# GlassyWing/yolo_deepsort

Measured on AMD Instinct MI355X. Metric: end-to-end frames/sec (detect+ReID+assoc), 608x608, higher is better.
Workload: dtype f16x3

## Files before the change

### include/ydsort.h

```cpp
#ifndef YDSORT_H
#define YDSORT_H

#include <stddef.h>
#include <stdint.h>

#ifdef __cplusplus
extern "C" {
#endif

typedef struct yds_net yds_net;
typedef struct yds_reid yds_reid;
typedef struct yds_trk yds_trk;
typedef struct yds_pipe yds_pipe;
typedef struct yds_zones yds_zones;
typedef struct yds_act yds_act;
typedef struct yds_ident yds_ident;
typedef struct yds_comm yds_comm;

int yds_init(int device_id);
int yds_current_device(void);
int yds_device_pci_bus_id(char *buf, int len);
const char *yds_last_error(void);
int yds_device_count(void);
const char *yds_build_info(void);
// ... 119 lines not shown
yds_pipe *yds_pipeline_create_multi(yds_net *, yds_reid *, yds_trk *const *trks, int n_streams, float conf_thres, float nms_thres,
                                    const int32_t *class_mask, int n_mask);
int yds_pipeline_step_multi(yds_pipe *, const uint8_t *frames_dev, const uint8_t *next_frames_dev, int h, int w, int n_frames,
                            const int32_t *stream_of_frame, int32_t *out6_host, int cap, int32_t *counts_host);
int yds_pipeline_step_multi_host(yds_pipe *, const uint8_t *frames_host, const uint8_t *next_frames_host, int h, int w, int n_frames,
                                 const int32_t *stream_of_frame, int32_t *out6_host, int cap, int32_t *counts_host);
int yds_pipeline_step_multi_mixed(yds_pipe *, const uint8_t *frames_dev, const uint8_t *next_frames_dev, const uint64_t *frame_off,
                                  const int32_t *frame_hw , size_t frames_bytes, int n_frames,
                                  const int32_t *stream_of_frame, int32_t *out6_host, int cap, int32_t *counts_host);
int yds_pipeline_step_multi_mixed_host(yds_pipe *, const uint8_t *frames_host, const uint8_t *next_frames_host, const uint64_t *frame_off,
                                       const int32_t *frame_hw , size_t frames_bytes, int n_frames,
                                       const int32_t *stream_of_frame, int32_t *out6_host, int cap, int32_t *counts_host);
int yds_pipeline_prefetch_host(yds_pipe *, const uint8_t *frames_host, int h, int w, int batch);
int yds_pipeline_set_schedule(yds_pipe *, int min_crops);
int yds_pipeline_set_frame_order(yds_pipe *, int bgr);
int yds_pipeline_set_windows(yds_pipe *, int win_w, int win_h, double overlap);
int yds_pipeline_set_stream_windows(yds_pipe *, int stream, int win_w, int win_h, double overlap);
int yds_pipeline_last_schedule(yds_pipe *);
int yds_pipeline_schedule_trial(yds_pipe *, int uploaded, int *decided, double *serialized_s, double *two_stream_s);
int yds_pipeline_stage_us(yds_pipe *, float *us5);
int yds_overlay_tracks(const uint8_t *frames_dev, const int32_t *src_slot_host, int n_out, int h, int w, const int32_t *boxes_host,
                       const int32_t *box_ptr_host, const uint8_t *text_host, int n_text, const int32_t *fps_host,
                       const uint8_t *font_host, int n_glyphs, int thickness, int scale, uint8_t *out_dev, uint8_t *out_host);
int yds_swap_rb(uint8_t *frames_dev, size_t pixels);
int yds_overlay_tracks_bgr(uint8_t *frames_bgr_dev, int n_src, const int32_t *src_slot_host, int n_out, int h, int w, const int32_t *boxes_host,
                           const int32_t *box_ptr_host, const uint8_t *text_host, int n_text, const int32_t *fps_host,
                           const uint8_t *font_host, int n_glyphs, int thickness, int scale, uint8_t *out_host);
int yds_conv_timing(yds_net *, int mode, double *total_us, int64_t *launches, double *flops);
int yds_conv_timing_ex(yds_net *, int mode, double *total_us, int64_t *launches, double *flops, double *bytes, double *attainable_us);
int yds_conv_num_variants(void);
// ... 102 lines not shown
```

### yolo_deepsort_amd/_lib.py

```python

from __future__ import annotations

import ctypes as C
import os

import numpy as np

HERE = os.path.dirname(os.path.abspath(__file__))
_TAG = os.environ.get("YDS_BUILD_TAG", "")
LIB_PATH = os.path.join(HERE, "libydsort" + ("_" + _TAG if _TAG else "") + ".so")


class YdsError(RuntimeError):
    pass


_P = C.c_void_p
_I = C.c_int
_F = C.c_float
_SZ = C.c_size_t
_I64 = C.c_int64

SIGNATURES = {
    "yds_init": (_I, [_I]),
# ... 99 lines not shown
    "yds_pipeline_step_host": (_I, [_P, _P, _P, _I, _I, _I, _P, _I, _P]),
    "yds_pipeline_create_multi": (_P, [_P, _P, _P, _I, _F, _F, _P, _I]),
    "yds_pipeline_step_multi": (_I, [_P, _P, _P, _I, _I, _I, _P, _P, _I, _P]),
    "yds_pipeline_step_multi_host": (_I, [_P, _P, _P, _I, _I, _I, _P, _P, _I, _P]),
    "yds_pipeline_prefetch_host": (_I, [_P, _P, _I, _I, _I]),
    "yds_pipeline_set_next_injection": (_I, [_P, _I]),
    "yds_pipeline_stage_us": (_I, [_P, _P]),
    "yds_pipeline_set_schedule": (_I, [_P, _I]),
    "yds_pipeline_last_schedule": (_I, [_P]),
    "yds_pipeline_schedule_trial": (_I, [_P, _I, _P, _P, _P]),
    "yds_conv_timing": (_I, [_P, _I, _P, _P, _P]),
    "yds_overlay_tracks": (_I, [_P, _P, _I, _I, _I, _P, _P, _P, _I, _P, _P, _I, _I, _I, _P, _P]),
    "yds_swap_rb": (_I, [_P, _SZ]),
    "yds_overlay_tracks_bgr": (_I, [_P, _I, _P, _I, _I, _I, _P, _P, _P, _I, _P, _P, _I, _I, _I, _P]),
    "yds_pipeline_set_frame_order": (_I, [_P, _I]),
    "yds_pipeline_set_windows": (_I, [_P, _I, _I, C.c_double]),
    "yds_darknet_forward_u8_mixed_dev": (_I, [_P, _P, _P, _P, _SZ, _I]),
    "yds_reid_preprocess_mixed": (_I, [_P, _P, _P, _P, _I, _SZ, _P, _P, _I, _P]),
    "yds_reid_embed_mixed": (_I, [_P, _P, _P, _P, _I, _SZ, _P, _P, _I, _I, _P]),
    "yds_reid_front_fused": (_I, [_P]),
    "yds_reid_front_grid_crops": (_I, []),
    "yds_pipeline_step_multi_mixed": (_I, [_P, _P, _P, _P, _P, _SZ, _I, _P, _P, _I, _P]),
    "yds_pipeline_step_multi_mixed_host": (_I, [_P, _P, _P, _P, _P, _SZ, _I, _P, _P, _I, _P]),
    "yds_nms_ragged_pred": (_I, [_P, _SZ, _I, _I, _P, _P, _P, _P, _F, _F, _P, _I, _P]),
    "yds_pipeline_set_stream_windows": (_I, [_P, _I, _I, _I, C.c_double]),
    "yds_pipeline_slot_pred": (_I, [_P, _P, _SZ, _P]),
    "yds_gallery_search": (_I, [_P, _I, _P, _I, _I, _I, _F, _I, _P, _P, _P, _P]),
    "yds_gallery_search_dense": (_I, [_P, _I, _P, _I, _I, _P, _P, _P, _P, _I, _P]),
    "yds_gallery_link": (_I, [_P, _I, _I, _I, _I, _I, _F, _I, _P, _P, _P, _P]),
    "yds_tracker_get_gallery": (_I, [_P, _I, _P, _I, _P]),
# ... 193 lines not shown
```

### yolo_deepsort_amd/csrc/common.h

```cpp
#pragma once
#include <hip/hip_runtime.h>
#include <stdint.h>
#include <stdio.h>
#include <string>
#include <vector>
#include <stdexcept>

#include "slot_plan.h"

namespace yds {

void set_error(const std::string &msg);
struct Error : std::runtime_error {
    explicit Error(const std::string &m) : std::runtime_error(m) {}
};
[[noreturn]] void fail(const char *fmt, ...);
int bound_device();
void bind_thread();
hipStream_t make_stream(bool latency_role);

#define YDS_HIP(expr)                                                                          \
    do {                                                                                       \
        hipError_t _e = (expr);                                                                \
        if (_e != hipSuccess)                                                                  \
// ... 84 lines not shown
const char *conv_variant_name(int v);
double conv_flops(const ConvArgs &a);
double conv_bytes_io(const View &v);
double conv_bytes(const ConvArgs &a);

void launch_maxpool(const View &x, const View &y, int k, int stride, int pad, bool zero_pad_br, hipStream_t s);
void launch_upsample(const View &x, const View &y, int stride, hipStream_t s);
void launch_copy(const View &x, const View &y, hipStream_t s);
void launch_add(const View &a, const View &b, const View &y, hipStream_t s);
void launch_nchw_to_nhwc(const float *src_nchw, const View &y, int c_src, hipStream_t s);
void launch_nhwc_to_nchw(const View &x, float *dst_nchw, hipStream_t s);
void nhwc_to_host(const View &x, float *dst_nchw_host, hipStream_t s);
void launch_pack_h16(const float *src_f32, const View &y, hipStream_t s);
void launch_yolo_decode(const View &head, float *out, int total_boxes, int box_off, int num_classes,
                        const float *anchors_wh , int A, int img_h, int img_w, hipStream_t s);
void launch_inject(const View &head, int image, const float *rows_dev, int n, int head_index, int num_classes,
                   float logit, hipStream_t s);
void launch_inject_batch(const View &head, int batch, const float *table_dev, const int *offsets_dev, int max_rows, int head_index,
                         int num_classes, float logit, hipStream_t s);
void launch_resize_u8(const uint8_t *frames, int n, int h, int w, const View &y, hipStream_t s, bool bgr = false);
std::vector<FrameGeom> checked_layout(const uint64_t *frame_off, const int32_t *frame_hw, int n, size_t frames_bytes);
void launch_slot_resize(const uint8_t *frames, const SlotRec *slots, int n, const View &y, hipStream_t s, bool bgr);
void launch_slot_boxes(const float *pred, int n_boxes, int attrs, const SlotRec *slots, int n, float *dst, hipStream_t s);
struct ReidFront {
    const uint8_t *frames = nullptr;
    const FrameGeom *geom = nullptr;
    const int *boxes = nullptr;
    int h = 0, w = 0, bgr = 0;
};
void launch_crop_resize(const ReidFront &f, int D, const View &y, hipStream_t s);
// ... 7 lines not shown
```

### yolo_deepsort_amd/csrc/darknet.cpp

```cpp
#include "engine.h"
#include "h16.h"
#include "conv_common.h"

#include <math.h>
#include <stdlib.h>
#include <string.h>
#include <map>
#include <sstream>

namespace yds {

std::vector<CfgBlock> parse_cfg(const std::string &text) {
    std::vector<CfgBlock> blocks;
    std::istringstream in(text);
    std::string line;
    auto strip = [](std::string s) {
        size_t a = s.find_first_not_of(" \t\r\n"), b = s.find_last_not_of(" \t\r\n");
        return a == std::string::npos ? std::string() : s.substr(a, b - a + 1);
    };
    while (std::getline(in, line)) {
        if (line.empty() || line[0] == '#') continue;
        line = strip(line);
        if (line.empty()) fail("cfg: whitespace-only line (the reference parser rejects it too)");
        if (line[0] == '[') {
// ... 466 lines not shown
        l.tuned_batch = batch;
        l.tuned_math = mode;
    };
    for (const Step &st : plan(batch).steps) {
        if (st.kind > Step::CONV_BLOCK1) continue;
        if (st.kind == Step::CONV_STEM2 || st.kind == Step::CONV_BLOCK1) tune(st.layer - 1, false);
        tune(st.layer, st.kind == Step::CONV_MERGED);
    }
}

void Darknet::check_pass(int batch) const {
    if (batch < 1 || batch > batch_max) fail("forward: batch %d outside [1,%d]", batch, batch_max);
    if (math != conv_math()) fail("forward: this network was planned for conv math %d, current mode is %d (re-create it)", math, conv_math());
}

void Darknet::run_graph(int batch) {
    check_pass(batch);
    int lanes = getenv("YDS_DET_LANES") ? atoi(getenv("YDS_DET_LANES")) : 1;
    while (lanes > 1 && batch / lanes < 4) --lanes;
    if (lanes < 1) lanes = 1;
    if (lanes == 1) { run_lane(0, batch, stream); return; }
    while ((int)lane_streams.size() < lanes - 1) {
        hipStream_t st; hipEvent_t ev;
        YDS_HIP(hipStreamCreateWithFlags(&st, hipStreamNonBlocking));
        YDS_HIP(hipEventCreateWithFlags(&ev, hipEventDisableTiming));
        lane_streams.push_back(st); lane_done.push_back(ev);
    }
    if (!lane_fork) YDS_HIP(hipEventCreateWithFlags(&lane_fork, hipEventDisableTiming));
    const int per = (batch + lanes - 1) / lanes;
    YDS_HIP(hipEventRecord(lane_fork, stream));
    for (int k = 0; k < lanes; ++k) {
        const int first = k * per, cnt = std::min(per, batch - first);
        if (cnt <= 0) break;
        hipStream_t st = (k == 0 || time_convs) ? stream : lane_streams[k - 1];
        if (st != stream) YDS_HIP(hipStreamWaitEvent(st, lane_fork, 0));
        run_lane(first, cnt, st);
        if (st != stream) {
            YDS_HIP(hipEventRecord(lane_done[k - 1], st));
            YDS_HIP(hipStreamWaitEvent(stream, lane_done[k - 1], 0));
        }
    }
}

int Darknet::head_layers() const {
    double total = 0, acc = 0;
    for (int i = 0; i < (int)layers.size(); ++i)
        if (layers[i].type == L_CONV) total += conv_flops(conv_args(i, 1));
    for (int i = 0; i < (int)layers.size(); ++i) {
        if (layers[i].type != L_CONV) continue;
        acc += conv_flops(conv_args(i, 1));
        if (acc >= 0.06 * total) return i + 1;
    }
    return (int)layers.size();
}

bool Darknet::forward_resized_part(int batch, int part) {
    check_pass(batch);
    if (getenv("YDS_DET_LANES") && atoi(getenv("YDS_DET_LANES")) > 1) return false;
    const int cut = head_layers();
    if (part == 0) run_lane(0, batch, stream, 0, cut);
    else run_lane(0, batch, stream, cut, -1);
    return true;
}

void Darknet::enqueue_conv(const Step &st, int first, int batch, hipStream_t stream) {
    const int i = st.layer;
    const Layer &l = layers[i];
    if (!l.cw.loaded()) fail("forward: layer %d has no weights (call load_darknet_weights)", i);
    const ConvArgs a = conv_args(i, batch, first, st.kind == Step::CONV_MERGED);
    ConvTimeRec rec;
    if (time_convs) { rec.e0 = timing_event(); rec.e1 = timing_event(); YDS_HIP(hipEventRecord(rec.e0, stream)); }
    int variant;
    double extra_flops = 0, extra_bytes = 0;
    if (st.kind == Step::CONV_STEM2) {
        const ConvArgs a0 = conv_args(i - 1, batch, first);
        ConvKernelArgs k0 = make_conv_args(a0), k1 = make_conv_args(a);
// ... 13 lines not shown
        extra_bytes = conv_bytes(a2) - conv_bytes_io(a2.y) - conv_bytes_io(a.x) - (a.res.p ? conv_bytes_io(a.res) : 0.0);
    } else {
        variant = launch_conv(a, stream, l.variant);
    }
    if (time_convs) {
        YDS_HIP(hipEventRecord(rec.e1, stream));
        rec.variant = variant;
        rec.flops = conv_flops(a) + extra_flops;
        rec.bytes = conv_bytes(a) + extra_bytes;
        const double peak = conv_math() == MATH_F32 ? 157.3e12 : (a.terms == 1 ? 2500e12 : 2500e12 / 3);
        rec.attain_us = std::max(rec.flops / peak, rec.bytes / 6.29e12) * 1e6;
        conv_pending.push_back(rec);
    }
}

void Darknet::run_lane(int first, int batch, hipStream_t stream, int l0, int l1) {
    autotune(batch);
    if (l1 < 0) l1 = (int)layers.size();
    auto v = [&](int layer) { return view(layer, batch, first); };
    for (const Step &st : plan(batch).steps) {
        const int i = st.layer;
        if (i < l0) continue;
        if (i >= l1) break;
        const Layer &l = layers[i];
        switch (st.kind) {
        case Step::CONV: case Step::CONV_MERGED: case Step::CONV_STEM2: case Step::CONV_BLOCK1:
            enqueue_conv(st, first, batch, stream);
            break;
        case Step::MAXPOOL: launch_maxpool(v(st.src), v(i), st.ksize, st.stride, st.pad, st.zero_br, stream); break;
        case Step::UPSAMPLE: launch_upsample(v(l.src), v(i), l.stride, stream); break;
        case Step::COPY: {
// ... 1 lines not shown
            d.p += fmt_slots(d.fmt, st.arg);
            launch_copy(v(st.src), d, stream);
            break;
        }
        case Step::ADD: launch_add(v(l.refs[0]), v(l.refs[1]), v(i), stream); break;
        case Step::YOLO: {
            const View head = v(l.src);
            const int hidx = st.arg;
            if (inject_active && inject_set >= 0) {
                launch_inject_batch(head, batch, inject_table.p, inject_offsets_dev.p + (size_t)inject_set * batch_max + first, inject_max_rows, hidx,
                                    l.classes, inject_logit, stream);
            } else {
                for (int b = 0; b < batch && inject_active; ++b)
                    launch_inject(head, b, inject_rows[first + b].p, inject_n[first + b], hidx, l.classes, inject_logit, stream);
            }
            launch_yolo_decode(head, out.p + (size_t)first * total_boxes * attrs, total_boxes, l.box_off, l.classes, l.anchors.data(), (int)l.anchors.size() / 2, img_h, img_w, stream);
            break;
        }
        }
    }
}

void Darknet::forward_f32_host(const float *nchw, int batch, float *out_host) {
    size_t n = (size_t)batch * in_channels * img_h * img_w;
    YDS_HIP(hipMemcpyAsync(stage_f32.p, nchw, n * sizeof(float), hipMemcpyHostToDevice, stream));
    launch_nchw_to_nhwc(stage_f32.p, input_view(batch), in_channels, stream);
    run_graph(batch);
    if (out_host) YDS_HIP(hipMemcpyAsync(out_host, out.p, (size_t)batch * total_boxes * attrs * sizeof(float), hipMemcpyDeviceToHost, stream));
    YDS_HIP(hipStreamSynchronize(stream));
}

// ... 291 lines not shown
```

### yolo_deepsort_amd/csrc/engine.h

```cpp
#pragma once
#include "common.h"
#include "conv_weights.h"

#include <map>
#include <memory>
#include <string>
#include <utility>
#include <vector>

namespace yds {

struct CfgBlock {
    std::string type;
    std::map<std::string, std::string> kv;
};
std::vector<CfgBlock> parse_cfg(const std::string &text);

enum LayerType { L_CONV, L_MAXPOOL, L_UPSAMPLE, L_ROUTE, L_SHORTCUT, L_YOLO };

struct Layer {
    LayerType type = L_CONV;
    int c = 0, h = 0, w = 0;
    int root = -1, coff = 0;
    int src = -1;
// ... 26 lines not shown
    std::vector<Step> steps;
    std::vector<int> produced_by;
    int batch = -1, math = -1, epoch = -1;
};

struct Storage {
    DevBuf<float> buf;
    int ld = 0;
    int fmt = 0;
    int fmt_half = 0;
    bool owns = false;
    bool redirected = false;
    int into = -1, coff = 0;
};

class Darknet {
public:
    Darknet(const std::string &cfg_text, int img_h, int img_w, int batch_max);
    ~Darknet();
    void load_weights(const void *blob, size_t nbytes, int cutoff);
    void set_batch_max(int b);
    void forward_f32_host(const float *nchw, int batch, float *out_host);
    void forward_u8_host(const uint8_t *frames, int h, int w, int batch, float *out_host);
    void forward_u8_dev(const uint8_t *frames_dev, int h, int w, int batch);
    void forward_u8_frames_dev(const uint8_t *frames_dev, const std::vector<FrameGeom> &geom);
    void forward_resized(int batch) { run_graph(batch); }
    bool forward_resized_part(int batch, int part);
    int head_layers() const;
    void forward_tiles_host(const uint8_t *frame, int h, int w, const int *tiles_xyhw, int n_tiles);
    void forward_slots(const uint8_t *frames_dev, const SlotRec *slots, int n_slots, float *pred, bool bgr);
    void layer_output_host(int layer, int batch, float *nchw);
    void get_input_host(int batch, float *nchw);
    void set_injection(int image, const float *rows, int n, float logit);
    void load_injection_sets(const float *rows, const int *offsets, int n_sets, float logit);
    void select_injection_set(int set);
    void enable_conv_timing(bool on);
    void autotune(int batch);
    int64_t flops_per_image() const;
    View view(int layer, int batch, int first = 0) const;
    View input_view(int batch, int first = 0) const;
    ConvArgs conv_args(int layer, int batch, int first = 0, bool merged = false) const;

// ... 22 lines not shown
    int inject_max_rows = 0;
    int inject_set = -1;
    float inject_logit = 6.f;
    struct ConvTimeRec { hipEvent_t e0 = nullptr, e1 = nullptr; int variant = 0; double flops = 0, bytes = 0, attain_us = 0; };
    bool time_convs = false;
    std::vector<ConvTimeRec> conv_pending;
    std::vector<hipEvent_t> ev_pool;
    hipEvent_t timing_event();
    void resolve_conv_timing();
    double conv_us[kConvVariants] = {}, conv_flops_acc[kConvVariants] = {}, conv_bytes_acc[kConvVariants] = {}, conv_attain_us[kConvVariants] = {};
    int64_t conv_launches[kConvVariants] = {};

private:
    void allocate_buffers();
    void check_pass(int batch) const;
    void run_graph(int batch);
    void run_lane(int first, int batch, hipStream_t st, int l0 = 0, int l1 = -1);
    void enqueue_conv(const Step &st, int first, int batch, hipStream_t s);
    const LaunchPlan &plan(int batch);
    LaunchPlan plan_;
    int plan_epoch = 0;
    bool stem_fusable = false;
    int block1_at = -1;
    std::vector<hipStream_t> lane_streams;
    std::vector<hipEvent_t> lane_done;
    hipEvent_t lane_fork = nullptr;
};

struct NmsUniform { int32_t n_boxes, corner, merge; float sx, sy; };
class NmsWorkspace {
public:
    explicit NmsWorkspace(int max_candidates = 16384, int frames = 1);
    ~NmsWorkspace();
    NmsWorkspace(const NmsWorkspace &) = delete;
    void launch(const float *pred_dev, const NmsUniform &u, int n_frames, int attrs, float conf_thres, float iou_thres, int cap, hipStream_t s);
    void launch(const float *pred_dev, const NmsFrame *fr, int n_frames, int max_rows, size_t total_rows, int attrs, float conf_thres,
                float iou_thres, int cap, hipStream_t s);
    int collect(int frame, float *out6_host, int cap);
    void resize(int max_candidates, int n_frames);
    int needed(int n_frames) const;
    static constexpr int kMaxCandidates = 1 << 18;
    int run(const float *pred_dev, int n_boxes, int attrs, float conf_thres, float iou_thres, float sx, float sy,
            float *out6_host, int cap, hipStream_t s);
    int run_merge(const float *pred_dev, int n_boxes, int attrs, float conf_thres, float iou_thres, float *out6_host, int cap, hipStream_t s);
    int max_cand, frames;
    DevBuf<float> cand;
    DevBuf<float> sorted;
    DevBuf<int> counts;
    DevBuf<int> box_count;
    DevBuf<unsigned long long> mask;
    DevBuf<float> kept;
    int *h_counts = nullptr;
// ... 117 lines not shown
```

### yolo_deepsort_amd/csrc/layers.hip

```cpp
#include "common.h"

#include <algorithm>
#include "h16.h"
#include "resize_dev.h"

namespace yds {

static inline int grid_for(size_t work, int block = 256) {
    size_t g = (work + block - 1) / block;
    if (g > 8192) g = 8192;
    if (g < 1) g = 1;
    return (int)g;
}

__global__ void maxpool_kernel(const float *x, float *y, int N, int H, int W, int C, int ldx, int Ho, int Wo, int ldy,
                               int k, int stride, int pad, int zero_br, int fmt_in, int fmt_out) {
    fp16_saturate_on();
    const int C4 = C >> 2;
    const size_t total = (size_t)N * Ho * Wo * C4;
    for (size_t idx = blockIdx.x * (size_t)blockDim.x + threadIdx.x; idx < total; idx += (size_t)gridDim.x * blockDim.x) {
        int c4 = idx % C4;
        size_t pix = idx / C4;
        int ox = pix % Wo;
        size_t t = pix / Wo;
// ... 153 lines not shown
    if (y.c % 32 || y.ld % 32) fail("pack_h16: channels must be a multiple of 32");
    hipLaunchKernelGGL(pack_h16_kernel, dim3(grid_for(y.pixels() * (y.c / 4))), dim3(256), 0, s, src_f32, y.p, y.pixels(), y.c, y.ld);
    YDS_HIP(hipGetLastError());
}

void launch_nhwc_to_nchw(const View &x, float *dst_nchw, hipStream_t s) {
    hipLaunchKernelGGL(nhwc_to_nchw_kernel, dim3(grid_for(x.pixels() * x.c)), dim3(256), 0, s, x.p, dst_nchw, x.n, x.c, x.h, x.w, x.ld, x.fmt);
    YDS_HIP(hipGetLastError());
}

struct YoloParams {
    float aw[8], ah[8];
    float s0, s1;
};

__global__ void yolo_decode_kernel(const float *head, float *out, int N, int H, int W, int ld, int A, int attrs, int total_boxes,
                                   int box_off, YoloParams yp) {
    const int HW = H * W, n = blockIdx.y, per_cell = A * attrs;
    (void)N;
    const int lane = threadIdx.x & 63;
    const int wave0 = __builtin_amdgcn_readfirstlane((int)((blockIdx.x * blockDim.x + threadIdx.x) >> 6));
    const int nwaves = (int)((gridDim.x * blockDim.x) >> 6);
    for (int cell = wave0; cell < HW; cell += nwaves) {
        const int gy = cell / W, gx = cell - gy * W;
        const float *src = head + ((size_t)(n * H + gy) * W + gx) * ld;
        float *dst = out + ((size_t)n * total_boxes + box_off + cell) * attrs;
        for (int i = lane; i < per_cell; i += 64) {
            int a = 0;
#pragma unroll
            for (int k = 1; k < 8; ++k) a += (k < A && i >= k * attrs) ? 1 : 0;
            const int t = i - a * attrs;
            const float v = src[i];
            float r;
            if (t == 0) r = __fmul_rn(__fadd_rn(1.f / (1.f + expf(-v)), (float)gx), yp.s0);
            else if (t == 1) r = __fmul_rn(__fadd_rn(1.f / (1.f + expf(-v)), (float)gy), yp.s1);
            else if (t == 2) r = __fmul_rn(__fmul_rn(expf(v), yp.aw[a]), yp.s0);
            else if (t == 3) r = __fmul_rn(__fmul_rn(expf(v), yp.ah[a]), yp.s1);
            else r = 1.f / (1.f + expf(-v));
            dst[(size_t)a * HW * attrs + t] = r;
        }
    }
}

void launch_yolo_decode(const View &head, float *out, int total_boxes, int box_off, int num_classes, const float *anchors_wh,
                        int A, int img_h, int img_w, hipStream_t s) {
    if (A > 8) fail("yolo: at most 8 anchors per head");
    YoloParams yp;
    yp.s0 = (float)((double)img_h / head.h);
    yp.s1 = (float)((double)img_w / head.w);
    for (int a = 0; a < A; ++a) {
        yp.aw[a] = anchors_wh[2 * a] / yp.s0;
        yp.ah[a] = anchors_wh[2 * a + 1] / yp.s1;
    }
    int attrs = num_classes + 5;
    if (head.c != A * attrs) fail("yolo: head has %d channels, expected %d", head.c, A * attrs);
    const size_t per_img = (size_t)A * head.h * head.w * attrs;
    if (per_img >= (1ull << 31)) fail("yolo: head too large for 32-bit indexing");
    const unsigned cells = (unsigned)head.h * head.w;
    hipLaunchKernelGGL(yolo_decode_kernel, dim3(std::min((cells + 3) / 4, 2048u), head.n), dim3(256), 0, s, head.p, out, head.n, head.h, head.w,
                       head.ld, A, attrs, total_boxes, box_off, yp);
    YDS_HIP(hipGetLastError());
}

__global__ void inject_clear_kernel(float *head, int image, int H, int W, int ld, int A, int attrs, float logit) {
    int total = H * W * A;
    for (int idx = blockIdx.x * blockDim.x + threadIdx.x; idx < total; idx += gridDim.x * blockDim.x) {
        int a = idx % A, cell = idx / A;
        head[((size_t)image * H * W + cell) * ld + a * attrs + 4] = -logit;
    }
}
__device__ __forceinline__ bool inject_row_superseded(const float *rows, int r, int n) {
    const float *row = rows + (size_t)r * 9;
    for (int j = r + 1; j < n; ++j) {
        const float *o = rows + (size_t)j * 9;
        if (o[0] == row[0] && o[1] == row[1] && o[2] == row[2] && o[3] == row[3]) return true;
// ... 202 lines not shown
```

### yolo_deepsort_amd/csrc/nms.hip

```cpp
#include "engine.h"

#include <string.h>

#include <vector>

namespace yds {

constexpr int MAX_DET = 300;

__device__ __forceinline__ NmsFrame frame_at(const NmsUniform &u, int f) {
    return NmsFrame{(uint64_t)f * u.n_boxes, u.n_boxes, u.corner, u.merge, u.sx, u.sy, 0};
}
__device__ __forceinline__ NmsFrame frame_at(const NmsFrame *fr, int f) { return fr[f]; }

__device__ __forceinline__ void nms_count_body(const float *pred, int n_boxes, int attrs, float thr, int *box_count) {
    int i = blockIdx.x * blockDim.x + threadIdx.x;
    if (i >= n_boxes) return;
    const float *p = pred + (size_t)i * attrs;
    int cnt = 0;
    float obj = p[4];
    if (obj > thr) {
        for (int j = 5; j < attrs; ++j) cnt += __fmul_rn(p[j], obj) > thr;
    }
    box_count[i] = cnt;
// ... 244 lines not shown
    if (!frame_at(frames, blockIdx.x).merge) return;
    nms_merge_body(cand_all, sorted_all, counts_all, max_cand, iou_thres, kept_all);
}

__global__ __launch_bounds__(256) void nms_publish_kernel(const int *counts, const float *kept, int *h_counts, float *h_kept, int cap) {
    const int f = blockIdx.x;
    if (threadIdx.x < 4) h_counts[f * 4 + threadIdx.x] = counts[f * 4 + threadIdx.x];
    const int n = min(counts[f * 4 + 1], cap) * 6;
    const float *src = kept + (size_t)f * MAX_DET * 6;
    float *dst = h_kept + (size_t)f * MAX_DET * 6;
    for (int i = threadIdx.x; i < n; i += 256) dst[i] = src[i];
}

template <class Frames>
static void launch_stages(NmsWorkspace &w, const float *pred_dev, Frames frames, int n_frames, int max_rows, size_t total_rows, bool merge, int attrs,
                          float conf_thres, float iou_thres, int cap, hipStream_t s) {
    if (attrs < 6) fail("nms: predictions need at least one class");
    if (n_frames < 1 || max_rows < 1) fail("nms: %d frames of at most %d rows", n_frames, max_rows);
    if (n_frames > w.frames) w.resize(w.max_cand, n_frames);
    w.box_count.ensure(total_rows);
    const int nb = (max_rows + 255) / 256, max_cand = w.max_cand, words_ld = max_cand / 64;
    hipLaunchKernelGGL(nms_count_kernel<Frames>, dim3(nb, n_frames), dim3(256), 0, s, pred_dev, frames, attrs, conf_thres, w.box_count.p);
    hipLaunchKernelGGL(nms_scan_kernel<Frames>, dim3(1, n_frames), dim3(1024), 0, s, w.box_count.p, frames, w.counts.p);
    hipLaunchKernelGGL(nms_emit_kernel<Frames>, dim3(nb, n_frames), dim3(256), 0, s, pred_dev, frames, attrs, conf_thres, w.box_count.p, max_cand,
                       w.cand.p);
    hipLaunchKernelGGL(nms_rank_kernel, dim3(16, n_frames), dim3(256), 0, s, w.cand.p, w.counts.p, max_cand, w.sorted.p);
    hipLaunchKernelGGL(nms_mask_kernel, dim3(64, n_frames), dim3(256), 0, s, w.sorted.p, w.counts.p, max_cand, (double)iou_thres, w.mask.p, words_ld);
    hipLaunchKernelGGL(nms_sweep_kernel<Frames>, dim3(1, n_frames), dim3(256), words_ld * sizeof(unsigned long long), s, w.sorted.p, w.mask.p, words_ld,
                       w.counts.p, max_cand, frames, w.kept.p, cap);
    if (merge)
        hipLaunchKernelGGL(nms_merge_kernel<Frames>, dim3(n_frames), dim3(256), 0, s, w.cand.p, w.sorted.p, w.counts.p, max_cand, iou_thres, frames,
                           w.kept.p);
    hipLaunchKernelGGL(nms_publish_kernel, dim3(n_frames), dim3(256), 0, s, w.counts.p, w.kept.p, w.h_counts, w.h_kept, std::min(cap, (int)MAX_DET));
    YDS_HIP(hipGetLastError());
}

void NmsWorkspace::launch(const float *pred_dev, const NmsUniform &u, int n_frames, int attrs, float conf_thres, float iou_thres, int cap,
                          hipStream_t s) {
    launch_stages(*this, pred_dev, u, n_frames, u.n_boxes, (size_t)std::max(frames, n_frames) * u.n_boxes, u.merge != 0, attrs, conf_thres,
                  iou_thres, cap, s);
}

void NmsWorkspace::launch(const float *pred_dev, const NmsFrame *fr, int n_frames, int max_rows, size_t total_rows, int attrs, float conf_thres,
                          float iou_thres, int cap, hipStream_t s) {
    launch_stages(*this, pred_dev, fr, n_frames, max_rows, total_rows, true, attrs, conf_thres, iou_thres, cap, s);
}

template <class Launch> static void launch_grown(NmsWorkspace &w, int n_frames, hipStream_t s, Launch launch) {
    launch();
    YDS_HIP(hipStreamSynchronize(s));
    if (w.needed(n_frames) <= w.max_cand) return;
    w.resize(w.needed(n_frames), w.frames);
    launch();
    YDS_HIP(hipStreamSynchronize(s));
}

int NmsWorkspace::collect(int frame, float *out6_host, int cap) {
    const int *c = h_counts + frame * 4;
    if (c[0] > max_cand) fail("nms: %d candidates exceed the workspace capacity %d (caller must resize and relaunch)", c[0], max_cand);
    int n = c[1] < cap ? c[1] : cap;
// ... 113 lines not shown
```

### yolo_deepsort_amd/csrc/pipeline.cpp

```cpp
#include "engine.h"

#include <limits.h>
#include <stdlib.h>
#include <string.h>

#include <algorithm>
#include <chrono>
#include <utility>

namespace yds {

struct DetSlot {
    std::unique_ptr<NmsWorkspace> nms;
    hipEvent_t e0, e1, e2, e_nms;
    hipEvent_t e_r0, e_r1;
    bool reid_in_pass = false;
    DetSlot() { for (hipEvent_t *e : {&e0, &e1, &e2, &e_nms, &e_r0, &e_r1}) YDS_HIP(hipEventCreate(e)); }
    ~DetSlot() {
        for (hipEvent_t e : {e0, e1, e2, e_nms, e_r0, e_r1}) (void)hipEventDestroy(e);
        if (plan_tab) (void)hipHostFree(plan_tab);
    }
    void *plan_tab = nullptr;
    size_t plan_bytes = 0, plan_slots_n = 0;
    const SlotRec *plan_slots() const { return static_cast<const SlotRec *>(plan_tab); }
// ... 164 lines not shown
        p.split = false;
        if (!p.plan.empty()) s.write_plan(p.plan);
        if (p.plan.windowed) {
            YDS_HIP(hipEventRecord(s.e1, net->stream));
            return;
        }
        if (p.plan.direct()) launch_slot_resize(p.frames, s.plan_slots(), p.batch, net->input_view(p.batch), net->stream, frames_bgr);
        else launch_resize_u8(p.frames, p.batch, p.geo.h, p.geo.w, net->input_view(p.batch), net->stream, frames_bgr);
        YDS_HIP(hipEventRecord(s.e1, net->stream));
        stager.mark_read(p.frames, net->stream, FrameStager::DET);
        p.split = split && net->forward_resized_part(p.batch, 0);
    }
    void launch_detector_tail(Pass &p) {
        DetSlot &s = det[p.slot];
        const size_t per_slot = (size_t)net->total_boxes * net->attrs, n_slots = p.plan.slots.size();
        if (p.plan.windowed) {
            if (win_pred.n < n_slots * per_slot) {
                YDS_HIP(hipStreamSynchronize(net->stream));
                win_pred.alloc(n_slots * per_slot);
            }
            pred_rows = n_slots * net->total_boxes;
            net->forward_slots(p.frames, s.plan_slots(), (int)n_slots, win_pred.p, frames_bgr);
            stager.mark_read(p.frames, net->stream, FrameStager::DET);
        } else if (p.split) {
            (void)net->forward_resized_part(p.batch, 1);
        } else {
            net->forward_resized(p.batch);
        }
        YDS_HIP(hipEventRecord(s.e2, net->stream));
        if (p.plan.empty()) {
            const float sx = box_scale(p.geo.w, net->img_w), sy = box_scale(p.geo.h, net->img_h);
            s.nms->launch(net->out.p, NmsUniform{net->total_boxes, 0, 0, sx, sy}, p.batch, net->attrs, conf, nms_thres, 300, net->stream);
        } else {
            s.nms->launch(p.plan.windowed ? win_pred.p : net->out.p, s.plan_frames(), p.batch, p.plan.max_rows, n_slots * net->total_boxes,
                          net->attrs, conf, nms_thres, 300, net->stream);
        }
        YDS_HIP(hipEventRecord(s.e_nms, net->stream));
        p.done = Pass::WHOLE;
    }

    void set_windows(int ww, int wh, double overlap) {
        if (pending.frames || ahead.reid_in_flight) fail("pipeline: set_windows while a look-ahead pass is in flight (consume it with a step first)");
        if (ww > 0 && wh <= 0) fail("pipeline: window %d x %d", ww, wh);
        if (ww > 0 && !(overlap >= 0)) fail("pipeline: window overlap %g", overlap);
        if (ww > 0 && any_stream_windows()) fail("pipeline: set_windows while a stream holds a window setting of its own (set_stream_windows): one or the other");
        win_w = ww > 0 ? ww : 0; win_h = ww > 0 ? wh : 0; win_overlap = overlap;
    }
    bool any_stream_windows() const {
        for (const WindowSetting &sw : stream_win)
            if (sw.w > 0) return true;
        return false;
    }
    void set_stream_windows(int stream, int ww, int wh, double overlap) {
        if (!multi) fail("pipeline: created by yds_pipeline_create: it has no streams (window mode: yds_pipeline_set_windows)");
        if (stream < 0 || stream >= (int)trks.size()) fail("pipeline: stream %d outside [0,%zu)", stream, trks.size());
        if (ww > 0 && wh <= 0) fail("pipeline: window %d x %d", ww, wh);
        if (ww > 0 && !(overlap >= 0)) fail("pipeline: window overlap %g", overlap);
        if (pending.frames || ahead.reid_in_flight)
            fail("pipeline: set_stream_windows while a look-ahead pass is in flight (consume it with a step first)");
        if (win_w > 0) fail("pipeline: set_stream_windows while window mode is on for all streams (yds_pipeline_set_windows): one or the other");
        stream_win.resize(trks.size());
// ... 249 lines not shown
    const int deep_min;
    DetSlot det[2];
    Pass pending;
    FrameStager stager;
    Dets cur, ahead;
    DevBuf<float> feat_cur;
    int next_inject_set = -1;
    hipEvent_t ev_feat = nullptr;
    int schedule_min_crops = INT_MIN;
    Trial trials[2];
    hipEvent_t ev_reid_done = nullptr;
    hipStream_t reid_last_on = nullptr;
    bool last_serial = false;
    bool frames_bgr = false;
    float stage_us[5] = {0, 0, 0, 0, 0};
    int win_w = 0, win_h = 0;
    double win_overlap = 0;
    DevBuf<float> win_pred;
    std::vector<WindowSetting> stream_win;
    size_t pred_rows = 0;
};

}

struct yds_pipe { yds::Pipeline *p; };

static void pipeline_step(yds_pipe *p, bool multi_entry, bool host, const uint8_t *frames, const uint8_t *next_frames, int h, int w, int n,
                          const int32_t *stream_of_frame, int32_t *out6_host, int cap, int32_t *counts_host) {
    if (multi_entry) p->p->set_streams(stream_of_frame, n);
    else if (p->p->multi) yds::fail("pipeline: created by yds_pipeline_create_multi: use yds_pipeline_step_multi%s", host ? "_host" : "");
// ... 83 lines not shown
int yds_pipeline_prefetch_host(yds_pipe *p, const uint8_t *frames_host, int h, int w, int batch) {
    YDS_API_BEGIN
    p->p->prefetch_host(frames_host, h, w, batch);
    YDS_API_END
}
int yds_pipeline_set_next_injection(yds_pipe *p, int set) {
    YDS_API_BEGIN
    p->p->next_inject_set = set;
    YDS_API_END
}
int yds_pipeline_set_frame_order(yds_pipe *p, int bgr) {
    YDS_API_BEGIN
    p->p->frames_bgr = bgr != 0;
    YDS_API_END
}
int yds_pipeline_set_windows(yds_pipe *p, int win_w, int win_h, double overlap) {
    YDS_API_BEGIN
    p->p->set_windows(win_w, win_h, overlap);
    YDS_API_END
}
int yds_pipeline_set_stream_windows(yds_pipe *p, int stream, int win_w, int win_h, double overlap) {
    YDS_API_BEGIN
    p->p->set_stream_windows(stream, win_w, win_h, overlap);
    YDS_API_END
}
int yds_pipeline_set_actions(yds_pipe *p, yds_act *a) {
    YDS_API_BEGIN
    p->p->set_actions(a ? a->a : nullptr);
    YDS_API_END
}
// ... 76 lines not shown
```

### yolo_deepsort_amd/pipeline.py

```python

from __future__ import annotations

import ctypes as C

import numpy as np

from . import _lib


def _refuse_tracker_nms(deepsort, message):
    if getattr(deepsort, "nms_max_overlap", 1) != 1:
        raise ValueError(message % (deepsort.nms_max_overlap,))


def _check_host_frames(frames, next_frames=None):
    assert frames.dtype == np.uint8 and frames.ndim == 4 and frames.flags["C_CONTIGUOUS"]
    if next_frames is not None:
        assert next_frames.shape == frames.shape and next_frames.dtype == np.uint8 and next_frames.flags["C_CONTIGUOUS"]
    return frames.shape[:3]


def pack_frames(frames):
    frames = [np.asarray(f) for f in frames]
    for i, f in enumerate(frames):
# ... 27 lines not shown
    def __init__(self, net, deepsort, conf_thres=0.5, nms_thres=0.4, class_mask=None, cap=512, win_size=None, overlap=0.15):
        self.net, self.ds, self.cap = net, deepsort, int(cap)
        self._h = None
        _refuse_tracker_nms(deepsort, "Pipeline: DeepSort(nms_max_overlap=%r) needs the frame-by-frame path (DeepSort.update / "
                                      "VideoDetector(batch_frames=1)); the batched pipeline has no tracker-side NMS")
        mask = np.ascontiguousarray(class_mask if class_mask is not None else [], dtype=np.int32)
        self._h = _lib.check_ptr(_lib.load().yds_pipeline_create(net._h, deepsort.extractor._h, deepsort.tracker._h,
                                                                 conf_thres, nms_thres,
                                                                 _lib.ptr(mask) if mask.size else None, int(mask.size)))
        self.set_windows(win_size, overlap)

    def set_windows(self, win_size=None, overlap=0.15):
        ww, wh = (0, 0) if win_size is None else (int(win_size[0]), int(win_size[1]))
        _lib.check(_lib.load().yds_pipeline_set_windows(self._h, ww, wh, float(overlap)))
        self.win_size, self.overlap = (None if win_size is None else (ww, wh)), overlap

    def step(self, frames_dev, h, w, batch, next_frames_dev=None, select_next=None):
        return self._run(batch, select_next, lambda out, counts: _lib.load().yds_pipeline_step(
            self._h, frames_dev, next_frames_dev, h, w, batch, out, self.cap, counts))

    def _run(self, n, select_next, call, streams=None):
        self._zone_streams = None if streams is None else [int(v) for v in streams]
        out = np.zeros((n, self.cap, 6), np.int32)
        counts = np.zeros(n, np.int32)
        if select_next is not None:
            _lib.check(_lib.load().yds_pipeline_set_next_injection(self._h, int(select_next)))
        _lib.check(call(_lib.ptr(out), _lib.ptr(counts)))
        self._last_counts = counts
        return [None if counts[b] < 0 else out[b, :counts[b]].copy() for b in range(n)]

# ... 296 lines not shown
```

Before: 1685.

## Gate YOLO decode on objectness and fuse NMS candidate counting into decode

Adds a sparse YOLO decode kernel that first evaluates objectness per box, fully decodes only boxes above the confidence threshold, and writes per-box candidate counts directly. The NMS stage then skips its separate count kernel when these counts are supplied. This targets the work of decoding every attribute of every box and a separate pass over predictions. In exchange, rows below threshold keep only objectness written, which is correct only if downstream readers check objectness first. The kernel also uses shared-memory atomics and extra block synchronisation per 64-box group.

```diff
diff --git a/include/ydsort.h b/include/ydsort.h
--- a/include/ydsort.h
+++ b/include/ydsort.h
@@ -157,6 +157,7 @@
 int yds_pipeline_prefetch_host(yds_pipe *, const uint8_t *frames_host, int h, int w, int batch);
 int yds_pipeline_set_schedule(yds_pipe *, int min_crops);
 int yds_pipeline_set_frame_order(yds_pipe *, int bgr);
+int yds_pipeline_set_dense_decode(yds_pipe *, int on);
 int yds_pipeline_set_windows(yds_pipe *, int win_w, int win_h, double overlap);
 int yds_pipeline_set_stream_windows(yds_pipe *, int stream, int win_w, int win_h, double overlap);
 int yds_pipeline_last_schedule(yds_pipe *);
diff --git a/yolo_deepsort_amd/_lib.py b/yolo_deepsort_amd/_lib.py
--- a/yolo_deepsort_amd/_lib.py
+++ b/yolo_deepsort_amd/_lib.py
@@ -137,6 +137,7 @@
     "yds_swap_rb": (_I, [_P, _SZ]),
     "yds_overlay_tracks_bgr": (_I, [_P, _I, _P, _I, _I, _I, _P, _P, _P, _I, _P, _P, _I, _I, _I, _P]),
     "yds_pipeline_set_frame_order": (_I, [_P, _I]),
+    "yds_pipeline_set_dense_decode": (_I, [_P, _I]),
     "yds_pipeline_set_windows": (_I, [_P, _I, _I, C.c_double]),
     "yds_darknet_forward_u8_mixed_dev": (_I, [_P, _P, _P, _P, _SZ, _I]),
     "yds_reid_preprocess_mixed": (_I, [_P, _P, _P, _P, _I, _SZ, _P, _P, _I, _P]),
diff --git a/yolo_deepsort_amd/csrc/common.h b/yolo_deepsort_amd/csrc/common.h
--- a/yolo_deepsort_amd/csrc/common.h
+++ b/yolo_deepsort_amd/csrc/common.h
@@ -122,6 +122,8 @@
 void launch_pack_h16(const float *src_f32, const View &y, hipStream_t s);
 void launch_yolo_decode(const View &head, float *out, int total_boxes, int box_off, int num_classes,
                         const float *anchors_wh , int A, int img_h, int img_w, hipStream_t s);
+void launch_yolo_decode_sparse(const View &head, float *out, int *box_count, float thr, int total_boxes, int box_off, int num_classes,
+                               const float *anchors_wh , int A, int img_h, int img_w, hipStream_t s);
 void launch_inject(const View &head, int image, const float *rows_dev, int n, int head_index, int num_classes,
                    float logit, hipStream_t s);
 void launch_inject_batch(const View &head, int batch, const float *table_dev, const int *offsets_dev, int max_rows, int head_index,
diff --git a/yolo_deepsort_amd/csrc/darknet.cpp b/yolo_deepsort_amd/csrc/darknet.cpp
--- a/yolo_deepsort_amd/csrc/darknet.cpp
+++ b/yolo_deepsort_amd/csrc/darknet.cpp
@@ -504,12 +504,12 @@
     if (math != conv_math()) fail("forward: this network was planned for conv math %d, current mode is %d (re-create it)", math, conv_math());
 }
 
-void Darknet::run_graph(int batch) {
+void Darknet::run_graph(int batch, DecodeGate gate) {
     check_pass(batch);
     int lanes = getenv("YDS_DET_LANES") ? atoi(getenv("YDS_DET_LANES")) : 1;
     while (lanes > 1 && batch / lanes < 4) --lanes;
     if (lanes < 1) lanes = 1;
-    if (lanes == 1) { run_lane(0, batch, stream); return; }
+    if (lanes == 1) { run_lane(0, batch, stream, 0, -1, gate); return; }
     while ((int)lane_streams.size() < lanes - 1) {
         hipStream_t st; hipEvent_t ev;
         YDS_HIP(hipStreamCreateWithFlags(&st, hipStreamNonBlocking));
@@ -524,7 +524,7 @@
         if (cnt <= 0) break;
         hipStream_t st = (k == 0 || time_convs) ? stream : lane_streams[k - 1];
         if (st != stream) YDS_HIP(hipStreamWaitEvent(st, lane_fork, 0));
-        run_lane(first, cnt, st);
+        run_lane(first, cnt, st, 0, -1, gate);
         if (st != stream) {
             YDS_HIP(hipEventRecord(lane_done[k - 1], st));
             YDS_HIP(hipStreamWaitEvent(stream, lane_done[k - 1], 0));
@@ -544,12 +544,12 @@
     return (int)layers.size();
 }
 
-bool Darknet::forward_resized_part(int batch, int part) {
+bool Darknet::forward_resized_part(int batch, int part, DecodeGate gate) {
     check_pass(batch);
     if (getenv("YDS_DET_LANES") && atoi(getenv("YDS_DET_LANES")) > 1) return false;
     const int cut = head_layers();
-    if (part == 0) run_lane(0, batch, stream, 0, cut);
-    else run_lane(0, batch, stream, cut, -1);
+    if (part == 0) run_lane(0, batch, stream, 0, cut, gate);
+    else run_lane(0, batch, stream, cut, -1, gate);
     return true;
 }
 
@@ -593,7 +593,7 @@
     }
 }
 
-void Darknet::run_lane(int first, int batch, hipStream_t stream, int l0, int l1) {
+void Darknet::run_lane(int first, int batch, hipStream_t stream, int l0, int l1, DecodeGate gate) {
     autotune(batch);
     if (l1 < 0) l1 = (int)layers.size();
     auto v = [&](int layer) { return view(layer, batch, first); };
@@ -625,7 +625,12 @@
                 for (int b = 0; b < batch && inject_active; ++b)
                     launch_inject(head, b, inject_rows[first + b].p, inject_n[first + b], hidx, l.classes, inject_logit, stream);
             }
-            launch_yolo_decode(head, out.p + (size_t)first * total_boxes * attrs, total_boxes, l.box_off, l.classes, l.anchors.data(), (int)l.anchors.size() / 2, img_h, img_w, stream);
+            float *rows = out.p + (size_t)first * total_boxes * attrs;
+            if (gate.box_count)
+                launch_yolo_decode_sparse(head, rows, gate.box_count + (size_t)first * total_boxes, gate.thr, total_boxes, l.box_off, l.classes,
+                                          l.anchors.data(), (int)l.anchors.size() / 2, img_h, img_w, stream);
+            else
+                launch_yolo_decode(head, rows, total_boxes, l.box_off, l.classes, l.anchors.data(), (int)l.anchors.size() / 2, img_h, img_w, stream);
             break;
         }
         }
diff --git a/yolo_deepsort_amd/csrc/engine.h b/yolo_deepsort_amd/csrc/engine.h
--- a/yolo_deepsort_amd/csrc/engine.h
+++ b/yolo_deepsort_amd/csrc/engine.h
@@ -64,6 +64,11 @@
     int into = -1, coff = 0;
 };
 
+struct DecodeGate {
+    float thr = 0.f;
+    int *box_count = nullptr;
+};
+
 class Darknet {
 public:
     Darknet(const std::string &cfg_text, int img_h, int img_w, int batch_max);
@@ -74,8 +79,8 @@
     void forward_u8_host(const uint8_t *frames, int h, int w, int batch, float *out_host);
     void forward_u8_dev(const uint8_t *frames_dev, int h, int w, int batch);
     void forward_u8_frames_dev(const uint8_t *frames_dev, const std::vector<FrameGeom> &geom);
-    void forward_resized(int batch) { run_graph(batch); }
-    bool forward_resized_part(int batch, int part);
+    void forward_resized(int batch, DecodeGate gate = DecodeGate()) { run_graph(batch, gate); }
+    bool forward_resized_part(int batch, int part, DecodeGate gate = DecodeGate());
     int head_layers() const;
     void forward_tiles_host(const uint8_t *frame, int h, int w, const int *tiles_xyhw, int n_tiles);
     void forward_slots(const uint8_t *frames_dev, const SlotRec *slots, int n_slots, float *pred, bool bgr);
@@ -128,8 +133,8 @@
 private:
     void allocate_buffers();
     void check_pass(int batch) const;
-    void run_graph(int batch);
-    void run_lane(int first, int batch, hipStream_t st, int l0 = 0, int l1 = -1);
+    void run_graph(int batch, DecodeGate gate = DecodeGate());
+    void run_lane(int first, int batch, hipStream_t st, int l0 = 0, int l1 = -1, DecodeGate gate = DecodeGate());
     void enqueue_conv(const Step &st, int first, int batch, hipStream_t s);
     const LaunchPlan &plan(int batch);
     LaunchPlan plan_;
@@ -147,9 +152,11 @@
     explicit NmsWorkspace(int max_candidates = 16384, int frames = 1);
     ~NmsWorkspace();
     NmsWorkspace(const NmsWorkspace &) = delete;
-    void launch(const float *pred_dev, const NmsUniform &u, int n_frames, int attrs, float conf_thres, float iou_thres, int cap, hipStream_t s);
+    void launch(const float *pred_dev, const NmsUniform &u, int n_frames, int attrs, float conf_thres, float iou_thres, int cap, hipStream_t s,
+                bool counted = false);
     void launch(const float *pred_dev, const NmsFrame *fr, int n_frames, int max_rows, size_t total_rows, int attrs, float conf_thres,
-                float iou_thres, int cap, hipStream_t s);
+                float iou_thres, int cap, hipStream_t s, bool counted = false);
+    int *counts_for(size_t total_rows) { box_count.ensure(total_rows); return box_count.p; }
     int collect(int frame, float *out6_host, int cap);
     void resize(int max_candidates, int n_frames);
     int needed(int n_frames) const;
diff --git a/yolo_deepsort_amd/csrc/layers.hip b/yolo_deepsort_amd/csrc/layers.hip
--- a/yolo_deepsort_amd/csrc/layers.hip
+++ b/yolo_deepsort_amd/csrc/layers.hip
@@ -191,6 +191,14 @@
     float s0, s1;
 };
 
+__device__ __forceinline__ float yolo_value(int t, float v, int a, int gx, int gy, const YoloParams &yp) {
+    if (t == 0) return __fmul_rn(__fadd_rn(1.f / (1.f + expf(-v)), (float)gx), yp.s0);
+    if (t == 1) return __fmul_rn(__fadd_rn(1.f / (1.f + expf(-v)), (float)gy), yp.s1);
+    if (t == 2) return __fmul_rn(__fmul_rn(expf(v), yp.aw[a]), yp.s0);
+    if (t == 3) return __fmul_rn(__fmul_rn(expf(v), yp.ah[a]), yp.s1);
+    return 1.f / (1.f + expf(-v));
+}
+
 __global__ void yolo_decode_kernel(const float *head, float *out, int N, int H, int W, int ld, int A, int attrs, int total_boxes,
                                    int box_off, YoloParams yp) {
     const int HW = H * W, n = blockIdx.y, per_cell = A * attrs;
@@ -207,20 +215,76 @@
 #pragma unroll
             for (int k = 1; k < 8; ++k) a += (k < A && i >= k * attrs) ? 1 : 0;
             const int t = i - a * attrs;
-            const float v = src[i];
-            float r;
-            if (t == 0) r = __fmul_rn(__fadd_rn(1.f / (1.f + expf(-v)), (float)gx), yp.s0);
-            else if (t == 1) r = __fmul_rn(__fadd_rn(1.f / (1.f + expf(-v)), (float)gy), yp.s1);
-            else if (t == 2) r = __fmul_rn(__fmul_rn(expf(v), yp.aw[a]), yp.s0);
-            else if (t == 3) r = __fmul_rn(__fmul_rn(expf(v), yp.ah[a]), yp.s1);
-            else r = 1.f / (1.f + expf(-v));
-            dst[(size_t)a * HW * attrs + t] = r;
-        }
-    }
-}
-
-void launch_yolo_decode(const View &head, float *out, int total_boxes, int box_off, int num_classes, const float *anchors_wh,
-                        int A, int img_h, int img_w, hipStream_t s) {
+            dst[(size_t)a * HW * attrs + t] = yolo_value(t, src[i], a, gx, gy, yp);
+        }
+    }
+}
+
+struct SparsePass { int lane, a, gx, gy, count; float obj; };
+__global__ __launch_bounds__(256) void yolo_decode_sparse_kernel(const float *__restrict__ head, float *__restrict__ out,
+                                                                 int *__restrict__ box_count, int H, int W, int ld, int A, int attrs,
+                                                                 int total_boxes, int box_off, float thr, YoloParams yp) {
+    __shared__ SparsePass passed[64];
+    __shared__ int n_passed;
+    const int HW = H * W, n = blockIdx.y, boxes = A * HW;
+    const int tid = threadIdx.x, lane = tid & 63;
+    const bool judge = tid < 64;
+    const float *img = head + (size_t)n * HW * ld;
+    const size_t row0 = (size_t)n * total_boxes + box_off;
+    for (int base = blockIdx.x * 64; base < boxes; base += gridDim.x * 64) {
+        const int box = base + lane;
+        bool pass = false;
+        int rank = 0;
+        if (judge) {
+            int a = 0, gx = 0, gy = 0;
+            float obj = 0.f;
+            if (box < boxes) {
+                a = box / HW;
+                const int cell = box - a * HW;
+                gy = cell / W; gx = cell - gy * W;
+                obj = yolo_value(4, img[(size_t)cell * ld + a * attrs + 4], a, gx, gy, yp);
+                pass = obj > thr;
+                if (!pass) {
+                    out[(row0 + box) * attrs + 4] = obj;
+                    box_count[row0 + box] = 0;
+                }
+            }
+            const unsigned long long m = __ballot(pass);
+            rank = __popcll(m & ((1ull << lane) - 1ull));
+            if (pass) passed[rank] = SparsePass{lane, a, gx, gy, 0, obj};
+            if (lane == 0) n_passed = __popcll(m);
+        }
+        __syncthreads();
+        const int total = n_passed * attrs;
+        for (int j = tid; j < total; j += 256 * 4) {
+            int ks[4], ts[4];
+            float v[4];
+#pragma unroll
+            for (int u = 0; u < 4; ++u) {
+                const int ju = j + 256 * u;
+                ks[u] = ju / attrs; ts[u] = ju - ks[u] * attrs;
+                v[u] = 0.f;
+                if (ju < total && ts[u] != 4) {
+                    const SparsePass &p = passed[ks[u]];
+                    v[u] = img[((size_t)p.gy * W + p.gx) * ld + p.a * attrs + ts[u]];
+                }
+            }
+#pragma unroll
+            for (int u = 0; u < 4; ++u) {
+                if (j + 256 * u >= total) continue;
+                const SparsePass &p = passed[ks[u]];
+                const float pobj = p.obj;
+                const float r = ts[u] == 4 ? pobj : yolo_value(ts[u], v[u], p.a, p.gx, p.gy, yp);
+                out[(row0 + base + p.lane) * attrs + ts[u]] = r;
+                if (ts[u] >= 5 && __fmul_rn(r, pobj) > thr) atomicAdd(&passed[ks[u]].count, 1);
+            }
+        }
+        __syncthreads();
+        if (pass) box_count[row0 + box] = passed[rank].count;
+    }
+}
+
+static YoloParams yolo_params(const View &head, int num_classes, const float *anchors_wh, int A, int img_h, int img_w) {
     if (A > 8) fail("yolo: at most 8 anchors per head");
     YoloParams yp;
     yp.s0 = (float)((double)img_h / head.h);
@@ -229,13 +293,28 @@
         yp.aw[a] = anchors_wh[2 * a] / yp.s0;
         yp.ah[a] = anchors_wh[2 * a + 1] / yp.s1;
     }
-    int attrs = num_classes + 5;
+    const int attrs = num_classes + 5;
     if (head.c != A * attrs) fail("yolo: head has %d channels, expected %d", head.c, A * attrs);
     const size_t per_img = (size_t)A * head.h * head.w * attrs;
     if (per_img >= (1ull << 31)) fail("yolo: head too large for 32-bit indexing");
+    return yp;
+}
+
+void launch_yolo_decode(const View &head, float *out, int total_boxes, int box_off, int num_classes, const float *anchors_wh,
+                        int A, int img_h, int img_w, hipStream_t s) {
+    const YoloParams yp = yolo_params(head, num_classes, anchors_wh, A, img_h, img_w);
     const unsigned cells = (unsigned)head.h * head.w;
     hipLaunchKernelGGL(yolo_decode_kernel, dim3(std::min((cells + 3) / 4, 2048u), head.n), dim3(256), 0, s, head.p, out, head.n, head.h, head.w,
-                       head.ld, A, attrs, total_boxes, box_off, yp);
+                       head.ld, A, num_classes + 5, total_boxes, box_off, yp);
+    YDS_HIP(hipGetLastError());
+}
+
+void launch_yolo_decode_sparse(const View &head, float *out, int *box_count, float thr, int total_boxes, int box_off, int num_classes,
+                               const float *anchors_wh, int A, int img_h, int img_w, hipStream_t s) {
+    const YoloParams yp = yolo_params(head, num_classes, anchors_wh, A, img_h, img_w);
+    const unsigned boxes = (unsigned)head.h * head.w * A;
+    hipLaunchKernelGGL(yolo_decode_sparse_kernel, dim3(std::min((boxes + 63) / 64, 2048u), head.n), dim3(256), 0, s, head.p, out, box_count,
+                       head.h, head.w, head.ld, A, num_classes + 5, total_boxes, box_off, thr, yp);
     YDS_HIP(hipGetLastError());
 }
 
diff --git a/yolo_deepsort_amd/csrc/nms.hip b/yolo_deepsort_amd/csrc/nms.hip
--- a/yolo_deepsort_amd/csrc/nms.hip
+++ b/yolo_deepsort_amd/csrc/nms.hip
@@ -282,13 +282,15 @@
 
 template <class Frames>
 static void launch_stages(NmsWorkspace &w, const float *pred_dev, Frames frames, int n_frames, int max_rows, size_t total_rows, bool merge, int attrs,
-                          float conf_thres, float iou_thres, int cap, hipStream_t s) {
+                          float conf_thres, float iou_thres, int cap, hipStream_t s, bool counted) {
     if (attrs < 6) fail("nms: predictions need at least one class");
     if (n_frames < 1 || max_rows < 1) fail("nms: %d frames of at most %d rows", n_frames, max_rows);
     if (n_frames > w.frames) w.resize(w.max_cand, n_frames);
+    if (counted && w.box_count.n < total_rows) fail("nms: a counted launch over %zu rows, counts_for() held %zu", total_rows, w.box_count.n);
     w.box_count.ensure(total_rows);
     const int nb = (max_rows + 255) / 256, max_cand = w.max_cand, words_ld = max_cand / 64;
-    hipLaunchKernelGGL(nms_count_kernel<Frames>, dim3(nb, n_frames), dim3(256), 0, s, pred_dev, frames, attrs, conf_thres, w.box_count.p);
+    if (!counted)
+        hipLaunchKernelGGL(nms_count_kernel<Frames>, dim3(nb, n_frames), dim3(256), 0, s, pred_dev, frames, attrs, conf_thres, w.box_count.p);
     hipLaunchKernelGGL(nms_scan_kernel<Frames>, dim3(1, n_frames), dim3(1024), 0, s, w.box_count.p, frames, w.counts.p);
     hipLaunchKernelGGL(nms_emit_kernel<Frames>, dim3(nb, n_frames), dim3(256), 0, s, pred_dev, frames, attrs, conf_thres, w.box_count.p, max_cand,
                        w.cand.p);
@@ -304,14 +306,14 @@
 }
 
 void NmsWorkspace::launch(const float *pred_dev, const NmsUniform &u, int n_frames, int attrs, float conf_thres, float iou_thres, int cap,
-                          hipStream_t s) {
+                          hipStream_t s, bool counted) {
     launch_stages(*this, pred_dev, u, n_frames, u.n_boxes, (size_t)std::max(frames, n_frames) * u.n_boxes, u.merge != 0, attrs, conf_thres,
-                  iou_thres, cap, s);
+                  iou_thres, cap, s, counted);
 }
 
 void NmsWorkspace::launch(const float *pred_dev, const NmsFrame *fr, int n_frames, int max_rows, size_t total_rows, int attrs, float conf_thres,
-                          float iou_thres, int cap, hipStream_t s) {
-    launch_stages(*this, pred_dev, fr, n_frames, max_rows, total_rows, true, attrs, conf_thres, iou_thres, cap, s);
+                          float iou_thres, int cap, hipStream_t s, bool counted) {
+    launch_stages(*this, pred_dev, fr, n_frames, max_rows, total_rows, true, attrs, conf_thres, iou_thres, cap, s, counted);
 }
 
 template <class Launch> static void launch_grown(NmsWorkspace &w, int n_frames, hipStream_t s, Launch launch) {
diff --git a/yolo_deepsort_amd/csrc/pipeline.cpp b/yolo_deepsort_amd/csrc/pipeline.cpp
--- a/yolo_deepsort_amd/csrc/pipeline.cpp
+++ b/yolo_deepsort_amd/csrc/pipeline.cpp
@@ -202,6 +202,9 @@
     void launch_detector_tail(Pass &p) {
         DetSlot &s = det[p.slot];
         const size_t per_slot = (size_t)net->total_boxes * net->attrs, n_slots = p.plan.slots.size();
+        const size_t nms_rows = p.plan.empty() ? (size_t)std::max(s.nms->frames, p.batch) * net->total_boxes : n_slots * net->total_boxes;
+        DecodeGate gate;
+        if (!dense_decode && !p.plan.windowed) gate = DecodeGate{conf, s.nms->counts_for(nms_rows)};
         if (p.plan.windowed) {
             if (win_pred.n < n_slots * per_slot) {
                 YDS_HIP(hipStreamSynchronize(net->stream));
@@ -211,17 +214,18 @@
             net->forward_slots(p.frames, s.plan_slots(), (int)n_slots, win_pred.p, frames_bgr);
             stager.mark_read(p.frames, net->stream, FrameStager::DET);
         } else if (p.split) {
-            (void)net->forward_resized_part(p.batch, 1);
+            (void)net->forward_resized_part(p.batch, 1, gate);
         } else {
-            net->forward_resized(p.batch);
+            net->forward_resized(p.batch, gate);
         }
         YDS_HIP(hipEventRecord(s.e2, net->stream));
+        const bool counted = gate.box_count != nullptr;
         if (p.plan.empty()) {
             const float sx = box_scale(p.geo.w, net->img_w), sy = box_scale(p.geo.h, net->img_h);
-            s.nms->launch(net->out.p, NmsUniform{net->total_boxes, 0, 0, sx, sy}, p.batch, net->attrs, conf, nms_thres, 300, net->stream);
+            s.nms->launch(net->out.p, NmsUniform{net->total_boxes, 0, 0, sx, sy}, p.batch, net->attrs, conf, nms_thres, 300, net->stream, counted);
         } else {
-            s.nms->launch(p.plan.windowed ? win_pred.p : net->out.p, s.plan_frames(), p.batch, p.plan.max_rows, n_slots * net->total_boxes,
-                          net->attrs, conf, nms_thres, 300, net->stream);
+            s.nms->launch(p.plan.windowed ? win_pred.p : net->out.p, s.plan_frames(), p.batch, p.plan.max_rows, nms_rows, net->attrs, conf,
+                          nms_thres, 300, net->stream, counted);
         }
         YDS_HIP(hipEventRecord(s.e_nms, net->stream));
         p.done = Pass::WHOLE;
@@ -233,6 +237,10 @@
         if (ww > 0 && !(overlap >= 0)) fail("pipeline: window overlap %g", overlap);
         if (ww > 0 && any_stream_windows()) fail("pipeline: set_windows while a stream holds a window setting of its own (set_stream_windows): one or the other");
         win_w = ww > 0 ? ww : 0; win_h = ww > 0 ? wh : 0; win_overlap = overlap;
+    }
+    void set_dense_decode(bool on) {
+        if (pending.frames || ahead.reid_in_flight) fail("pipeline: set_dense_decode while a look-ahead pass is in flight (consume it with a step first)");
+        dense_decode = on;
     }
     bool any_stream_windows() const {
         for (const WindowSetting &sw : stream_win)
@@ -512,6 +520,7 @@
     bool last_serial = false;
     bool frames_bgr = false;
     float stage_us[5] = {0, 0, 0, 0, 0};
+    bool dense_decode = getenv("YDS_DENSE_DECODE") && atoi(getenv("YDS_DENSE_DECODE"));
     int win_w = 0, win_h = 0;
     double win_overlap = 0;
     DevBuf<float> win_pred;
@@ -625,6 +634,11 @@
     p->p->frames_bgr = bgr != 0;
     YDS_API_END
 }
+int yds_pipeline_set_dense_decode(yds_pipe *p, int on) {
+    YDS_API_BEGIN
+    p->p->set_dense_decode(on != 0);
+    YDS_API_END
+}
 int yds_pipeline_set_windows(yds_pipe *p, int win_w, int win_h, double overlap) {
     YDS_API_BEGIN
     p->p->set_windows(win_w, win_h, overlap);
diff --git a/yolo_deepsort_amd/pipeline.py b/yolo_deepsort_amd/pipeline.py
--- a/yolo_deepsort_amd/pipeline.py
+++ b/yolo_deepsort_amd/pipeline.py
@@ -65,6 +65,9 @@
         ww, wh = (0, 0) if win_size is None else (int(win_size[0]), int(win_size[1]))
         _lib.check(_lib.load().yds_pipeline_set_windows(self._h, ww, wh, float(overlap)))
         self.win_size, self.overlap = (None if win_size is None else (ww, wh)), overlap
+
+    def set_dense_decode(self, on=True):
+        _lib.check(_lib.load().yds_pipeline_set_dense_decode(self._h, 1 if on else 0))
 
     def step(self, frames_dev, h, w, batch, next_frames_dev=None, select_next=None):
         return self._run(batch, select_next, lambda out, counts: _lib.load().yds_pipeline_step(
```

Result: no change. 1702, median of 6 (+1.0%).
